# zhoujun-7/VPHO

Measured on AMD Instinct MI355X. Metric: eval images/sec (bs=64, sample_num=100, steps=50); MPJPE delta vs ref, higher is better.
Workload: dtype f32; 1 GPU; vpho_net.forward(mode=predict), README eval config (BASELINE.json configs[1]); per_gpu_batch=64, sample_num=100, sampling_steps=50, topk_hand=30, topk_obj=10, crop=256x256, pipeline_depth=3, parallelism=dp1, score_mfma=f32, conv_mfma=f32, winograd_3x3=True

## Files before the change

vpho_amd/csrc/common.h:

```cpp
#pragma once
#include <hip/hip_runtime.h>
#include <cstdio>
#include <cstdarg>

namespace vpho {
char* err_slot();
int fail(const char* fmt, ...);
inline int check_launch(const char* what) {
    hipError_t e = hipGetLastError();
    if (e != hipSuccess) return fail("%s: %s", what, hipGetErrorString(e));
    return 0;
}

enum ProfClass { PROF_CONV128 = 0, PROF_CONV64 = 1, PROF_SCORE_HEAD = 2, PROF_CONV128x64 = 3,
                 PROF_MANO_FK = 4, PROF_OBJ_PHYSICS = 5, PROF_HAND_FUSE = 6, PROF_ROI_ALIGN = 7, PROF_RESIZE = 8, PROF_WINOGRAD = 9,
                 PROF_WGRAD64 = 10, PROF_WGRAD128 = 11, PROF_FORCE_OPTIM = 12, PROF_POSE_ENC = 13, PROF_NCLASS = 14 };
bool prof_on(int cls);
void prof_record(int cls, hipEvent_t start, hipEvent_t stop, double flops, double bytes);
struct ProfScope {
    int cls; hipStream_t s; double flops, bytes; bool on; hipEvent_t e0, e1;
    ProfScope(int c, hipStream_t st, double f, double b = 0) : cls(c), s(st), flops(f), bytes(b), on(c >= 0 && prof_on(c)) {
        if (on) { (void)hipEventCreate(&e0); (void)hipEventCreate(&e1); (void)hipEventRecord(e0, s); }
    }
    ~ProfScope() { if (on) { (void)hipEventRecord(e1, s); prof_record(cls, e0, e1, flops, bytes); } }
};
int dynamic_lds(const void* kernel, int bytes);
}

#define VPHO_REQUIRE(cond, ...) do { if (!(cond)) return vpho::fail(__VA_ARGS__); } while (0)
#define VPHO_DYN_LDS(kernel, bytes) do { if (vpho::dynamic_lds(reinterpret_cast<const void*>(kernel), (int)(bytes))) return 1; } while (0)
#define VPHO_HIP(call) do { hipError_t e_ = (call); if (e_ != hipSuccess) return vpho::fail("%s: %s", #call, hipGetErrorString(e_)); } while (0)

#define VPHO_SYNC_LDS_DMA() do { asm volatile("s_waitcnt vmcnt(0)" ::: "memory"); __syncthreads(); } while (0)
#define VPHO_BARRIER_LDS_ONLY() asm volatile("s_waitcnt lgkmcnt(0)\n\ts_barrier" ::: "memory")

#ifndef VPHO_MAINLOOP_PRIO
#define VPHO_MAINLOOP_PRIO 0
#endif
#if VPHO_MAINLOOP_PRIO
#define VPHO_PRIO_MAIN() __builtin_amdgcn_s_setprio(VPHO_MAINLOOP_PRIO)
#define VPHO_PRIO_REST() __builtin_amdgcn_s_setprio(0)
#else
#define VPHO_PRIO_MAIN() ((void)0)
#define VPHO_PRIO_REST() ((void)0)
#endif

__device__ inline void lin_src(int dst, float scale, int in_size, int& i0, int& i1, float& l1) {
    float s = ((float)dst + 0.5f) * scale - 0.5f;
    s = s < 0.f ? 0.f : s;
    i0 = (int)s;
    i1 = i0 + (i0 < in_size - 1 ? 1 : 0);
    l1 = s - (float)i0;
}

#ifdef VPHO_CLOCK_STAMPS
#define VPHO_STAMP_SLOTS 65536
#define VPHO_STAMP_WORDS 10
#define VPHO_STAMP_DECL(name)                                                                                                      \
    __device__ unsigned long long name##_stamps[VPHO_STAMP_WORDS * VPHO_STAMP_SLOTS];                                              \
// ... 56 lines not shown
```

vpho_amd/csrc/mano.hip:

```cpp
#include "common.h"
#include "rot.h"
#include "../../include/vpho_hip.h"

namespace {

__constant__ int c_parent[16] = {-1, 0, 1, 2, 0, 4, 5, 0, 7, 8, 0, 10, 11, 0, 13, 14};
__constant__ int c_tips[5] = {745, 317, 444, 556, 673};
__constant__ int c_tips_ho3d[5] = {728, 353, 442, 576, 694};
__constant__ int c_order[21] = {0, 13, 14, 15, 16, 1, 2, 3, 17, 4, 5, 6, 18, 10, 11, 12, 19, 7, 8, 9, 20};
__constant__ int c_to_manolayer[21] = {0, 5, 6, 7, 9, 10, 11, 17, 18, 19, 13, 14, 15, 1, 2, 3, 4, 8, 12, 16, 20};

constexpr int NV = 778;

__global__ __launch_bounds__(256) void mano_shape_kernel(const vpho_mano_tables t, const float* __restrict__ betas, int n_img,
                                                         float* __restrict__ v_shaped, float* __restrict__ J) {
    __shared__ float vs[NV * 3];
    __shared__ float be[10];
    const int b = blockIdx.x;
    if (threadIdx.x < 10) be[threadIdx.x] = betas[b * 10 + threadIdx.x];
    __syncthreads();
    for (int i = threadIdx.x; i < NV * 3; i += blockDim.x) {
        float s = 0.f;
        for (int k = 0; k < 10; ++k) s += t.shapedirs[i * 10 + k] * be[k];
        s += t.v_template[i];
        vs[i] = s;
        v_shaped[(long long)b * NV * 3 + i] = s;
    }
    __syncthreads();
    const int wave = threadIdx.x >> 6, lane = threadIdx.x & 63;
    for (int o = wave; o < 48; o += 4) {
        const int j = o / 3, c = o % 3;
        float s = 0.f;
        for (int v = lane; v < NV; v += 64) s += t.J_regressor[j * NV + v] * vs[v * 3 + c];
        for (int off = 32; off > 0; off >>= 1) s += __shfl_xor(s, off);
        if (lane == 0) J[b * 48 + o] = s;
    }
}

struct FkArgs {
    vpho_mano_tables t;
    const float* pose; int ld_pose;
    const float* v_shaped; const float* J;
    long long n_hands; int hands_per_image;
    const unsigned char* ho3d;
    float* verts;
    float* joints;
};

template <int HB>
__global__ __launch_bounds__(256) void mano_fk_kernel(const FkArgs a) {
    __shared__ float R[HB][16][9];
    __shared__ float G[HB][16][12];
    __shared__ __attribute__((aligned(16))) float A[HB][16][12];
    __shared__ __attribute__((aligned(16))) float pmT[135][HB];
    __shared__ float jt[HB][21][3];
    __shared__ float tipv[HB][10][3];
    const int tid = threadIdx.x;
    const long long h0 = (long long)blockIdx.x * HB;
    auto hand_of = [&](int h) { const long long g = h0 + h; return g < a.n_hands ? g : a.n_hands - 1; };
    auto img_of = [&](int h) { return (int)(hand_of(h) / a.hands_per_image); };
    const int hj_h = tid >> 4, hj_j = tid & 15;
    const bool hj = tid < HB * 16;

    if (hj) {
        float r[9];
        vpho::mano_rodrigues(a.pose + hand_of(hj_h) * a.ld_pose + 3 * hj_j, r);
        for (int k = 0; k < 9; ++k) R[hj_h][hj_j][k] = r[k];
    }
    __syncthreads();
    for (int i = tid; i < HB * 135; i += 256) {
        const int h = i / 135, k = i - h * 135;
        const int e = k % 9;
        pmT[k][h] = R[h][k / 9 + 1][e] - ((e == 0 || e == 4 || e == 8) ? 1.f : 0.f);
    }
    for (int lvl = 0; lvl < 4; ++lvl) {
        if (hj && (hj_j == 0 ? 0 : (hj_j - 1) % 3 + 1) == lvl) {
            const float* Jr = a.J + img_of(hj_h) * 48;
            const int i = hj_j;
            float (*Gh)[12] = G[hj_h];
            const float* Ri = R[hj_h][i];
            if (i == 0) {
                for (int k = 0; k < 3; ++k) { for (int c = 0; c < 3; ++c) Gh[0][k * 4 + c] = Ri[k * 3 + c]; Gh[0][k * 4 + 3] = Jr[k]; }
            } else {
                const int p = c_parent[i];
                const float rel[3] = {Jr[i * 3 + 0] - Jr[p * 3 + 0], Jr[i * 3 + 1] - Jr[p * 3 + 1], Jr[i * 3 + 2] - Jr[p * 3 + 2]};
                for (int r = 0; r < 3; ++r) {
                    for (int c = 0; c < 3; ++c) {
                        float s = 0.f;
                        for (int k = 0; k < 3; ++k) s += Gh[p][r * 4 + k] * Ri[k * 3 + c];
                        Gh[i][r * 4 + c] = s;
                    }
                    float s = 0.f;
                    for (int k = 0; k < 3; ++k) s += Gh[p][r * 4 + k] * rel[k];
                    Gh[i][r * 4 + 3] = s + Gh[p][r * 4 + 3];
                }
            }
        }
        __syncthreads();
    }
    if (hj) {
        const float* Jr = a.J + img_of(hj_h) * 48;
        const int i = hj_j;
        for (int r = 0; r < 3; ++r) {
            float s = 0.f;
            for (int k = 0; k < 3; ++k) s += G[hj_h][i][r * 4 + k] * Jr[i * 3 + k];
            for (int c = 0; c < 3; ++c) A[hj_h][i][r * 4 + c] = G[hj_h][i][r * 4 + c];
            A[hj_h][i][r * 4 + 3] = G[hj_h][i][r * 4 + 3] - s;
            jt[hj_h][i][r] = G[hj_h][i][r * 4 + 3];
        }
    }
    __syncthreads();

    typedef float f32x2 __attribute__((ext_vector_type(2)));
    auto skin_tail = [&](int h, int v, const float* wv, const float* blend, float* out3) {
        const float* vsh = a.v_shaped + (long long)img_of(h) * NV * 3;
        float vp[3];
        for (int c = 0; c < 3; ++c) vp[c] = vsh[v * 3 + c] + blend[c];
        f32x2 T[6];
#pragma unroll
        for (int e = 0; e < 6; ++e) T[e] = f32x2{0.f, 0.f};
#pragma unroll
        for (int j = 0; j < 16; ++j) {
            const f32x2 w = {wv[j], wv[j]};
            const f32x2* Aj = reinterpret_cast<const f32x2*>(A[h][j]);
#pragma unroll
            for (int e = 0; e < 6; ++e) T[e] = __builtin_elementwise_fma(Aj[e], w, T[e]);
        }
        for (int r = 0; r < 3; ++r) out3[r] = fmaf(T[2 * r][0], vp[0], fmaf(T[2 * r][1], vp[1], fmaf(T[2 * r + 1][0], vp[2], T[2 * r + 1][1])));
    };
    auto fin = [](float v, float c) { return ((v - c) * 1000.f) / 1000.f; };

    if (blockIdx.y == 0) {
        for (int t = tid; t < HB * 10; t += 256) {
            const int h = t / 10, tip = t - h * 10;
            const int v = tip < 5 ? c_tips[tip] : c_tips_ho3d[tip - 5];
            float blend[3], wv[16], o[3];
            for (int c = 0; c < 3; ++c) {
                float s = 0.f;
                const float* pd = a.t.tip_posedirs_t ? a.t.tip_posedirs_t + tip * 3 + c : a.t.posedirs_t + v * 3 + c;
                const long long ld = a.t.tip_posedirs_t ? 30 : (long long)NV * 3;
                for (int k = 0; k < 135; ++k) s = fmaf(pd[k * ld], pmT[k][h], s);
                blend[c] = s;
            }
            for (int j = 0; j < 16; ++j) wv[j] = a.t.weights[v * 16 + j];
            skin_tail(h, v, wv, blend, o);
            for (int c = 0; c < 3; ++c) tipv[h][tip][c] = o[c];
            if (tip < 5) for (int c = 0; c < 3; ++c) jt[h][16 + tip][c] = o[c];
        }
        __syncthreads();
        for (int t = tid; t < HB * 21; t += 256) {
            const int h = t / 21, q = t - h * 21;
            if (h0 + h >= a.n_hands) continue;
            const bool ho = a.ho3d && a.ho3d[img_of(h)];
            const float cx = jt[h][0][0], cy = jt[h][0][1], cz = jt[h][0][2];
            const float* src;
            if (!ho) src = jt[h][c_order[q]];
            else if (q >= 16) src = tipv[h][5 + q - 16];
            else src = jt[h][c_order[c_to_manolayer[q]]];
            float* jo = a.joints + ((h0 + h) * 21 + q) * 3;
            jo[0] = fin(src[0], cx); jo[1] = fin(src[1], cy); jo[2] = fin(src[2], cz);
        }
    }
    if (a.verts) {
        const int v = (blockIdx.y * 4 + (tid >> 6)) * 64 + (tid & 63);
        if (v < NV) {
            float acc[HB][3];
            const float* pd = a.t.posedirs_t + v * 3;
            if constexpr (HB % 2 == 0) {
                f32x2 ap[HB / 2][3];
#pragma unroll
                for (int h = 0; h < HB / 2; ++h) ap[h][0] = ap[h][1] = ap[h][2] = f32x2{0.f, 0.f};
#pragma unroll 3
                for (int k = 0; k < 135; ++k) {
                    const float p0 = pd[(long long)k * NV * 3], p1 = pd[(long long)k * NV * 3 + 1], p2 = pd[(long long)k * NV * 3 + 2];
                    const f32x2 q0 = {p0, p0}, q1 = {p1, p1}, q2 = {p2, p2};
                    const f32x2* m2 = reinterpret_cast<const f32x2*>(pmT[k]);
#pragma unroll
// ... 241 lines not shown
                }
            __builtin_amdgcn_sched_barrier(0);
            if (v < NV) {
#pragma unroll
                for (int i = 0; i < 16; ++i) {
                    const int h = (i >> 2) * 8 + lh * 4 + (i & 3);
                    const float o = fmaf(T[0][i], acc[0][i], fmaf(T[1][i], acc[1][i], fmaf(T[2][i], acc[2][i], T[3][i])));
                    if ((FK_ABLATE & 1) && o != 1.2345e-30f) continue;
                    if (h0 + h < a.n_hands) a.verts[((h0 + h) * NV + v) * 3 + r] = fin(o, cen[i]);
                }
            }
            __builtin_amdgcn_sched_barrier(0);
        }
    }
}

}

extern "C" int vpho_mano_shape_f32(const vpho_mano_tables* t, const float* betas, int n_img, float* v_shaped, float* J, void* stream) {
    VPHO_REQUIRE(t && t->v_template && t->shapedirs && t->J_regressor && betas && v_shaped && J && n_img > 0, "vpho_mano_shape_f32: bad argument");
    hipLaunchKernelGGL(mano_shape_kernel, dim3(n_img), dim3(256), 0, (hipStream_t)stream, *t, betas, n_img, v_shaped, J);
    return vpho::check_launch("mano_shape_kernel");
}

extern "C" int vpho_mano_fk_f32(const vpho_mano_tables* t, const float* pose, int ld_pose, long long n_hands, int hands_per_image,
                                const float* v_shaped, const float* J, const unsigned char* ho3d_per_image,
                                float* verts, float* joints, void* stream) {
    VPHO_REQUIRE(t && t->posedirs_t && t->weights && pose && v_shaped && J && joints && n_hands > 0 && hands_per_image > 0 && ld_pose >= 48,
                 "vpho_mano_fk_f32: bad argument");
    VPHO_REQUIRE(n_hands < (1ll << 31), "vpho_mano_fk_f32: too many hands");
    FkArgs a;
    a.t = *t; a.pose = pose; a.ld_pose = ld_pose; a.v_shaped = v_shaped; a.J = J; a.n_hands = n_hands;
    a.hands_per_image = hands_per_image; a.ho3d = ho3d_per_image; a.verts = verts; a.joints = joints;
    const unsigned gy = verts ? 4 : 1;
    vpho::ProfScope prof(vpho::PROF_MANO_FK, (hipStream_t)stream, 0.0,
                         (double)n_hands * (48 * 4 + 21 * 12 + (verts ? 778 * 12 : 0)) + (double)((n_hands + hands_per_image - 1) / hands_per_image) * (778 + 16) * 12);
    static const bool no_mfma = getenv("VPHO_MANO_MFMA") && atoi(getenv("VPHO_MANO_MFMA")) == 0;
    if (verts && t->posedirs_mfma && n_hands >= 4096 && hands_per_image >= MH / 2 && !no_mfma) {
        VPHO_DYN_LDS(mano_fk_mfma_kernel, sizeof(FkMfmaLds));
        hipLaunchKernelGGL(mano_fk_mfma_kernel, dim3((unsigned)((n_hands + MH - 1) / MH)), dim3(512), sizeof(FkMfmaLds), (hipStream_t)stream, a);
        return vpho::check_launch("mano_fk_mfma_kernel");
    }
    if (n_hands >= 1024) hipLaunchKernelGGL(mano_fk_kernel<16>, dim3((unsigned)((n_hands + 15) / 16), gy), dim3(256), 0, (hipStream_t)stream, a);
    else if (n_hands >= 128) hipLaunchKernelGGL(mano_fk_kernel<4>, dim3((unsigned)((n_hands + 3) / 4), gy), dim3(256), 0, (hipStream_t)stream, a);
    else hipLaunchKernelGGL(mano_fk_kernel<1>, dim3((unsigned)n_hands, gy), dim3(256), 0, (hipStream_t)stream, a);
    return vpho::check_launch("mano_fk_kernel");
}
```

vpho_amd/csrc/misc.hip:

```cpp
#include "common.h"
#include <cstdint>
#include "rot.h"
#include "../../include/vpho_hip.h"

namespace {

inline int nblocks(long long n, int bs = 256) { return (int)((n + bs - 1) / bs); }

__global__ void nchw_to_nhwc_kernel(const float* __restrict__ x, int N, int C, int H, int W, float* __restrict__ y, int ldy) {
    const long long i = (long long)blockIdx.x * blockDim.x + threadIdx.x;
    const long long total = (long long)N * H * W * ldy;
    if (i >= total) return;
    const int c = (int)(i % ldy);
    const long long p = i / ldy;
    const long long hw = (long long)H * W;
    const long long n = p / hw, r = p - n * hw;
    y[i] = c < C ? x[(n * C + c) * hw + r] : 0.f;
}

__global__ void nhwc_to_nchw_kernel(const float* __restrict__ x, int N, int H, int W, int C, int ldx, float* __restrict__ y) {
    const long long i = (long long)blockIdx.x * blockDim.x + threadIdx.x;
    const long long hw = (long long)H * W, total = (long long)N * C * hw;
    if (i >= total) return;
    const long long r = i % hw;
    const long long nc = i / hw;
    const int c = (int)(nc % C);
    const long long n = nc / C;
    y[i] = x[(n * hw + r) * ldx + c];
}

__global__ void maxpool_nhwc_kernel(const float* __restrict__ x, int N, int H, int W, int C, int k, int stride, int pad,
                                    int OH, int OW, float* __restrict__ y) {
    const long long i = (long long)blockIdx.x * blockDim.x + threadIdx.x;
    const long long total = (long long)N * OH * OW * C;
    if (i >= total) return;
    const int c = (int)(i % C);
    long long p = i / C;
    const int ox = (int)(p % OW); p /= OW;
    const int oy = (int)(p % OH);
    const long long n = p / OH;
    float m = -INFINITY;
    for (int r = 0; r < k; ++r) {
        const int iy = oy * stride - pad + r;
        if (iy < 0 || iy >= H) continue;
        for (int s = 0; s < k; ++s) {
            const int ix = ox * stride - pad + s;
            if (ix < 0 || ix >= W) continue;
            m = fmaxf(m, x[((n * H + iy) * W + ix) * C + c]);
        }
    }
    y[i] = m;
}


template <int V>
__device__ inline void ldv(const float* __restrict__ p, float (&o)[V]) {
    if constexpr (V == 4) { const f32x4 t = *reinterpret_cast<const f32x4*>(p); o[0] = t[0]; o[1] = t[1]; o[2] = t[2]; o[3] = t[3]; }
    else o[0] = *p;
}
template <int V>
__device__ inline void stv(float* __restrict__ p, const float (&v)[V]) {
    if constexpr (V == 4) { f32x4 t; t[0] = v[0]; t[1] = v[1]; t[2] = v[2]; t[3] = v[3]; *reinterpret_cast<f32x4*>(p) = t; }
    else *p = v[0];
}

template <int V>
__global__ void resize_bilinear_nhwc_kernel(const float* __restrict__ x, int N, int H, int W, int C, int ldx, int OH, int OW,
                                            float* __restrict__ y, int ldy, int c_off, int accumulate,
                                            const int* __restrict__ row_map, const int* __restrict__ row_count) {
    const long long i = (long long)blockIdx.x * blockDim.x + threadIdx.x;
    const int CV = C / V;
    const long long total = (long long)N * OH * OW * CV;
    if (i >= total) return;
    const int c = (int)(i % CV) * V;
    long long p = i / CV;
    if (row_map) {
        if (p >= *row_count) return;
        p = row_map[p];
    }
    const int ox = (int)(p % OW); p /= OW;
    const int oy = (int)(p % OH);
    const long long n = p / OH;
    int y0, y1, x0, x1; float ly, lx;
    lin_src(oy, (float)H / (float)OH, H, y0, y1, ly);
// ... 407 lines not shown
    float* o = out + row * ldo + 3 * j;
    o[0] = aa[0]; o[1] = aa[1]; o[2] = aa[2];
}

__global__ void append_betas_kernel(const float* __restrict__ betas, long long rows, long long rows_per_image, float* __restrict__ out, int ldo) {
    const long long i = (long long)blockIdx.x * blockDim.x + threadIdx.x;
    if (i >= rows * 10) return;
    const long long row = i / 10;
    const int k = (int)(i - row * 10);
    out[row * ldo + 48 + k] = betas[(row / rows_per_image) * 10 + k];
}

}

#define LAUNCH1D(kernel, total, stream, ...) \
    hipLaunchKernelGGL(kernel, dim3(nblocks(total)), dim3(256), 0, (hipStream_t)(stream), __VA_ARGS__)

extern "C" int vpho_nchw_to_nhwc_f32(const float* x, int N, int C, int H, int W, float* y, int ldy, void* stream) {
    VPHO_REQUIRE(x && y && N > 0 && C > 0 && H > 0 && W > 0 && ldy >= C, "vpho_nchw_to_nhwc_f32: bad argument");
    LAUNCH1D(nchw_to_nhwc_kernel, (long long)N * H * W * ldy, stream, x, N, C, H, W, y, ldy);
    return vpho::check_launch("nchw_to_nhwc_kernel");
}

extern "C" int vpho_nhwc_to_nchw_f32(const float* x, int N, int H, int W, int C, int ldx, float* y, void* stream) {
    VPHO_REQUIRE(x && y && N > 0 && C > 0 && H > 0 && W > 0 && ldx >= C, "vpho_nhwc_to_nchw_f32: bad argument");
    LAUNCH1D(nhwc_to_nchw_kernel, (long long)N * H * W * C, stream, x, N, H, W, C, ldx, y);
    return vpho::check_launch("nhwc_to_nchw_kernel");
}

extern "C" int vpho_maxpool_nhwc_f32(const float* x, int N, int H, int W, int C, int k, int stride, int pad, float* y, void* stream) {
    VPHO_REQUIRE(x && y && N > 0 && C > 0 && k > 0 && stride > 0 && pad >= 0 && 2 * pad <= k, "vpho_maxpool_nhwc_f32: bad argument");
    const int OH = (H + 2 * pad - k) / stride + 1, OW = (W + 2 * pad - k) / stride + 1;
    VPHO_REQUIRE(OH > 0 && OW > 0, "vpho_maxpool_nhwc_f32: empty output");
    LAUNCH1D(maxpool_nhwc_kernel, (long long)N * OH * OW * C, stream, x, N, H, W, C, k, stride, pad, OH, OW, y);
    return vpho::check_launch("maxpool_nhwc_kernel");
}

extern "C" int vpho_resize_bilinear_nhwc_f32(const float* x, int N, int H, int W, int C, int ldx, int OH, int OW,
                                             float* y, int ldy, int c_off, int accumulate, void* stream) {
    VPHO_REQUIRE(x && y && N > 0 && C > 0 && H > 0 && W > 0 && OH > 0 && OW > 0 && ldx >= C && ldy >= c_off + C && c_off >= 0,
                 "vpho_resize_bilinear_nhwc_f32: bad argument");
    vpho::ProfScope prof(vpho::PROF_RESIZE, (hipStream_t)stream, 0.0, 4.0 * N * C * ((double)H * W + (double)OH * OW * (accumulate ? 2 : 1)));
    if (C % 4 == 0 && ldx % 4 == 0 && ldy % 4 == 0 && c_off % 4 == 0 && ((uintptr_t)x | (uintptr_t)y) % 16 == 0)
        LAUNCH1D(resize_bilinear_nhwc_kernel<4>, (long long)N * OH * OW * (C / 4), stream, x, N, H, W, C, ldx, OH, OW, y, ldy, c_off, accumulate, (const int*)nullptr, (const int*)nullptr);
    else
        LAUNCH1D(resize_bilinear_nhwc_kernel<1>, (long long)N * OH * OW * C, stream, x, N, H, W, C, ldx, OH, OW, y, ldy, c_off, accumulate, (const int*)nullptr, (const int*)nullptr);
    return vpho::check_launch("resize_bilinear_nhwc_kernel");
}

extern "C" int vpho_resize_bilinear_rows_nhwc_f32(const float* x, int N, int H, int W, int C, int ldx, int OH, int OW, float* y, int ldy, int c_off,
                                                  int accumulate, const int* row_map, const int* row_count, int rows_hint, void* stream) {
    VPHO_REQUIRE(x && y && row_map && row_count && N > 0 && H > 0 && W > 0 && C > 0 && OH > 0 && OW > 0 && ldx >= C && ldy >= c_off + C && c_off >= 0,
                 "vpho_resize_bilinear_rows_nhwc_f32: bad argument");
    const double px = rows_hint > 0 ? (double)rows_hint : (double)N * OH * OW;
    vpho::ProfScope prof(vpho::PROF_RESIZE, (hipStream_t)stream, 0.0, 4.0 * C * ((double)N * H * W + px * (accumulate ? 2 : 1)));
    if (C % 4 == 0 && ldx % 4 == 0 && ldy % 4 == 0 && c_off % 4 == 0 && ((uintptr_t)x | (uintptr_t)y) % 16 == 0)
        LAUNCH1D(resize_bilinear_nhwc_kernel<4>, (long long)N * OH * OW * (C / 4), stream, x, N, H, W, C, ldx, OH, OW, y, ldy, c_off, accumulate, row_map, row_count);
    else
        LAUNCH1D(resize_bilinear_nhwc_kernel<1>, (long long)N * OH * OW * C, stream, x, N, H, W, C, ldx, OH, OW, y, ldy, c_off, accumulate, row_map, row_count);
    return vpho::check_launch("resize_bilinear_nhwc_kernel(rows)");
}

extern "C" int vpho_roi_align_nhwc_f32(const float* feat, int N, int H, int W, int C, const float* boxes, float spatial_scale,
                                       int out_size, const unsigned char* flip_w, float* out, int ldo, int c_off, void* stream) {
    VPHO_REQUIRE(feat && boxes && out && N > 0 && C > 0 && out_size > 0 && ldo >= c_off + C && c_off >= 0, "vpho_roi_align_nhwc_f32: bad argument");
    vpho::ProfScope prof(vpho::PROF_ROI_ALIGN, (hipStream_t)stream, 0.0, 4.0 * N * C * ((double)H * W + (double)out_size * out_size));
// ... 85 lines not shown
    return vpho_mha_dropout_f32(qkv, S, B, E, nhead, nullptr, out, stream);
}

extern "C" int vpho_add_layernorm_f32(const float* x, const float* r, const float* gamma, const float* beta, long long rows, int E,
                                      float eps, float* out, void* stream) {
    VPHO_REQUIRE(x && r && gamma && beta && out && rows > 0 && E > 0, "vpho_add_layernorm_f32: bad argument");
    hipLaunchKernelGGL(add_layernorm_kernel, dim3((unsigned)((rows + 3) / 4)), dim3(256), 0, (hipStream_t)stream, x, r, gamma, beta, rows, E, eps, out);
    return vpho::check_launch("add_layernorm_kernel");
}

extern "C" int vpho_force_local_f32(const float* scale, int ld_scale, const float* logits, int ld_logits, const float* anchor,
                                    float friction, long long rows, int group, int group_stride, int off_scale, int off_logits,
                                    float* out, void* stream) {
    VPHO_REQUIRE(scale && logits && anchor && out && rows > 0 && ld_scale >= 1 && ld_logits >= 8 && group > 0 && group_stride >= group,
                 "vpho_force_local_f32: bad argument");
    LAUNCH1D(force_local_kernel, rows, stream, scale, ld_scale, logits, ld_logits, anchor, friction, rows, group, group_stride, off_scale, off_logits, out);
    return vpho::check_launch("force_local_kernel");
}

extern "C" int vpho_rot6d_to_axis_angle_f32(const float* x, long long rows, int rot_per_row, int ldx, float* out, int ldo, void* stream) {
    VPHO_REQUIRE(x && out && rows > 0 && rot_per_row > 0 && ldx >= 6 * rot_per_row && ldo >= 3 * rot_per_row, "vpho_rot6d_to_axis_angle_f32: bad argument");
    LAUNCH1D(rot6d_to_aa_kernel, rows * rot_per_row, stream, x, rows * rot_per_row, rot_per_row, ldx, out, ldo);
    return vpho::check_launch("rot6d_to_aa_kernel");
}

extern "C" int vpho_append_betas_f32(const float* betas, long long rows, long long rows_per_image, float* out, int ldo, void* stream) {
    VPHO_REQUIRE(betas && out && rows > 0 && rows_per_image > 0 && ldo >= 58, "vpho_append_betas_f32: bad argument");
    LAUNCH1D(append_betas_kernel, rows * 10, stream, betas, rows, rows_per_image, out, ldo);
    return vpho::check_launch("append_betas_kernel");
}


constexpr int LIN64_MAXK = 4096;
__global__ __launch_bounds__(256) void linear_acc64_kernel(const float* __restrict__ x, int rows, int K, int ld_x, const float* __restrict__ w,
                                                           const float* __restrict__ bias, int N, float slope, float* __restrict__ y, int ld_y) {
    const int n = blockIdx.x, lane = threadIdx.x & 63, wave = threadIdx.x >> 6;
    float wr[LIN64_MAXK / 64];
    const int nk = (K + 63) >> 6;
#pragma unroll
    for (int i = 0; i < LIN64_MAXK / 64; ++i) { const int k = i * 64 + lane; wr[i] = (i < nk && k < K) ? w[(long long)n * K + k] : 0.f; }
    const double b = bias ? (double)bias[n] : 0.0;
    for (int r = wave; r < rows; r += 4) {
        const float* xr = x + (long long)r * ld_x;
        double s = 0.0;
#pragma unroll
        for (int i = 0; i < LIN64_MAXK / 64; ++i) { const int k = i * 64 + lane; if (i < nk && k < K) s += (double)xr[k] * (double)wr[i]; }
        for (int off = 32; off > 0; off >>= 1) s += __shfl_xor(s, off);
        if (lane == 0) { const double v = s + b; y[(long long)r * ld_y + n] = (float)(v > 0.0 ? v : v * (double)slope); }
    }
}

extern "C" int vpho_linear_acc64_f32(const float* x, int rows, int cin, int ld_x, const float* w, const float* bias, int cout, float out_slope,
                                     float* y, int ld_y, void* stream) {
    VPHO_REQUIRE(x && w && y && rows > 0 && cin > 0 && cin <= LIN64_MAXK && cout > 0 && ld_x >= cin && ld_y >= cout, "vpho_linear_acc64_f32: bad argument (cin <= %d)", LIN64_MAXK);
    hipLaunchKernelGGL(linear_acc64_kernel, dim3(cout), dim3(256), 0, (hipStream_t)stream, x, rows, cin, ld_x, w, bias, cout, out_slope, y, ld_y);
    return vpho::check_launch("linear_acc64_kernel");
}
```

vpho_amd/csrc/score_ode.hip:

```cpp
#include "common.h"
#include <type_traits>
#include "../../include/vpho_hip.h"
#include <cmath>
#include <cstdlib>
#include <cstring>
#include <vector>
#include <mutex>
#include <unordered_map>
#include <algorithm>

VPHO_STAMP_DECL(head)

namespace {

#ifndef HEAD_ABLATE
#define HEAD_ABLATE 0
#endif
constexpr int HB_K = 16;
constexpr double SIGMA_MIN = 0.01, SIGMA_MAX = 50.0;

struct TimeList { float t[8]; };

struct RkCtl {
    double t, h_abs, h, t_new, err, dense_h;
    double T0, tf, rtol, atol, max_step, g_scale;
    double d[4];
    double *te, *dense_p, *log;
    int done, accepted, rejected, parity, kswap, status;
    int next_idx, num_steps, dense_first, dense_last, dense_parity, dense_kswap;
    int n_accepted, n_rejected, nfev, n_log, log_cap, n_attempts;
    float ts[8], inv_std[8], coef[8];
};
__device__ __host__ inline int kslot(int j, int kswap) { return (kswap && (j == 0 || j == 6)) ? 6 - j : j; }
__device__ inline bool ctl_skip(const RkCtl* ctl, int mode) {
    if (!ctl || mode == 0) return false;
    const int d = ctl->done;
    return mode == 1 ? d != 0 : d == 0;
}
__global__ __launch_bounds__(256) void time_embed_kernel(const vpho_score_weights w, TimeList tl, int NH, float* __restrict__ ct_all,
                                                         const RkCtl* __restrict__ ctl, int ctl_mode) {
    __shared__ float emb[128], tf[128];
    const int tid = threadIdx.x;
    if (ctl_skip(ctl, ctl_mode)) return;
    const float t = (ctl && ctl_mode == 1) ? ctl->ts[blockIdx.y] : tl.t[blockIdx.y];
    float* ct = ct_all + (long long)blockIdx.y * NH;
    if (tid < 64) {
        float a = t * w.t_W[tid];
        a = a * 2.0f;
        a = a * 3.14159265358979323846f;
        emb[tid] = sinf(a);
        emb[tid + 64] = cosf(a);
    }
    __syncthreads();
    if (tid < 128) {
        float s = 0.f;
        for (int i = 0; i < 128; ++i) s += w.t_w[tid * 128 + i] * emb[i];
        s += w.t_b[tid];
        tf[tid] = s > 0.f ? s : 0.f;
    }
    __syncthreads();
    const int o = blockIdx.x * 256 + tid;
    if (o < NH) {
        float s = 0.f;
        for (int k = 0; k < 128; ++k) s += tf[k] * w.w1_t[(long long)k * NH + o];
        ct[o] = s;
    }
}

struct LinComb { double c[7]; int n; double h; };
struct KSlots { const float* p[7]; };

struct PoseEncArgs {
    const float* X; int Dp;
    const double* y; KSlots ks; int D; LinComb lc; double* ynew; int use_lc;
    const float *w0, *b0, *w2, *b2;
    float* out; int R;
    const RkCtl* ctl; int ctl_mode, write_ynew; const float* kbase; long long n_el; double *ybuf0, *ybuf1;
};
constexpr int PE_ROWS = 32, PE_H_LD = 260, PE_NST = 3, PE_STAGE = 256 * 32;
__device__ __attribute__((aligned(256))) float g_pe_zero_page[64];

__global__ __launch_bounds__(512) void pose_encoder_kernel(const PoseEncArgs a) {
    extern __shared__ __attribute__((aligned(1024))) float smem[];
    const int K1 = (a.Dp + 31) / 32 * 32, X_LD = K1 + 4;
    float* Ws = smem;
    float* H1 = Ws + PE_NST * PE_STAGE;
    float* Bs = H1 + PE_ROWS * PE_H_LD;
    float* Xs = Bs + 512;
    const int tid = threadIdx.x, lane = tid & 63, wave = tid >> 6, li = lane & 31, lh = lane >> 5;
    const int r0 = blockIdx.x * PE_ROWS;
    const int n1 = K1 / 32, nch = n1 + 8;
    if (ctl_skip(a.ctl, a.ctl_mode)) return;
    KSlots ks = a.ks;
    const double* yv = a.y;
    double* ynew = a.ynew;
    double lch = a.lc.h;
    if (a.ctl && a.ctl_mode == 1 && a.use_lc) {
// ... 1233 lines not shown
    ws.bytes = off;
    return ws;
}

int check_weights(const vpho_score_weights* w) {
    VPHO_REQUIRE(w != nullptr, "score weights: null");
    VPHO_REQUIRE(w->nheads > 0 && w->D == w->nheads * 3 && w->Dp >= w->D && w->Dp % 4 == 0, "score weights: D=%d Dp=%d nheads=%d inconsistent", w->D, w->Dp, w->nheads);
    VPHO_REQUIRE(w->t_W && w->t_w && w->t_b && w->pe0_w && w->pe0_b && w->pe2_w && w->pe2_b && w->w1_t && w->w1_p && w->w1_f && w->b1 && w->w2 && w->b2, "score weights: null tensor");
    return 0;
}

int linear(const float* x, int rows, int cin, const float* wt, const float* bias, int cout, float slope, float* y, hipStream_t s) {
    vpho_conv_desc d;
    memset(&d, 0, sizeof(d));
    d.x = x; d.w = wt; d.bias = bias; d.y = y;
    d.N = rows; d.H = 1; d.W = 1; d.Cin = cin; d.x_ld = cin; d.Cout = cout; d.KH = 1; d.KW = 1; d.stride = 1;
    d.OH = 1; d.OW = 1; d.y_sx = cout; d.y_sy = cout; d.y_sn = cout; d.in_slope = 1.f; d.out_slope = slope;
    return vpho_conv2d_nhwc_f32(&d, s);
}

float sigma_f32(float t) { return (float)SIGMA_MIN * (float)std::pow(SIGMA_MAX / SIGMA_MIN, (double)t); }

struct Ctx {
    const vpho_score_weights* w; Workspace ws; int bs, S; long long R, n_el; int NH; hipStream_t s;
};

int prepare_cimg(Ctx& c, const float* feat_img) {
    return linear(feat_img, c.bs, 1024, c.w->w1_f, c.w->b1, c.NH, 1.f, c.ws.cimg, c.s);
}

int embed_times(Ctx& c, const float* ts, int n, int ctl_mode = 0) {
    TimeList tl;
    for (int i = 0; i < 8; ++i) tl.t[i] = (ts && i < n) ? ts[i] : 0.f;
    hipLaunchKernelGGL(time_embed_kernel, dim3((c.NH + 255) / 256, n), dim3(256), 0, c.s, *c.w, tl, c.NH, c.ws.ct,
                       ctl_mode ? c.ws.ctl : (const RkCtl*)nullptr, ctl_mode);
    return vpho::check_launch("time_embed_kernel");
}

struct CtlCall { int mode = 0, stage = 0, out_slot = 0, write_ynew = 0; };

int eval_net(Ctx& c, const float* X, float t, int rhs_mode, float coef, float* out, int ct_slot = -1,
             const LinComb* lc = nullptr, const double* y = nullptr, double* ynew = nullptr, const KSlots* ks = nullptr,
             CtlCall cc = CtlCall()) {
    if (ct_slot < 0) {
        if (int e = embed_times(c, &t, 1, cc.mode == 2 ? 2 : 0)) return e;
        ct_slot = 0;
    }
    {
        PoseEncArgs pa;
        memset(&pa, 0, sizeof(pa));
        pa.X = X; pa.Dp = c.w->Dp; pa.w0 = c.w->pe0_w; pa.b0 = c.w->pe0_b; pa.w2 = c.w->pe2_w; pa.b2 = c.w->pe2_b;
        pa.out = c.ws.P2; pa.R = (int)c.R;
        if (lc) { pa.use_lc = 1; pa.lc = *lc; pa.y = y; if (ks) pa.ks = *ks; pa.D = c.w->D; pa.ynew = ynew; }
        pa.ctl = cc.mode ? c.ws.ctl : nullptr; pa.ctl_mode = cc.mode; pa.write_ynew = cc.write_ynew; pa.kbase = c.ws.K; pa.n_el = c.n_el;
        pa.ybuf0 = c.ws.y; pa.ybuf1 = c.ws.ynew;
        const int K1 = (pa.Dp + 31) / 32 * 32;
        const char* pe_env = getenv("VPHO_PE_RING");
        const bool pe_ring = pe_env && atoi(pe_env);
        const dim3 pe_grid((unsigned)((c.R + PE_ROWS - 1) / PE_ROWS));
        vpho::ProfScope pe_prof(vpho::PROF_POSE_ENC, c.s, 2.0 * (double)c.R * 256.0 * (K1 + 256.0), 0.0);
        if (pe_ring) {
            const size_t pe_lds = (size_t)(PE_NST * PE_STAGE + PE_ROWS * PE_H_LD + 512 + PE_ROWS * (K1 + 4)) * sizeof(float);
            VPHO_DYN_LDS(pose_encoder_kernel, 150 * 1024);
            VPHO_REQUIRE(pe_lds <= 150 * 1024, "pose encoder: input dimension %d too large for the LDS tile", pa.Dp);
            hipLaunchKernelGGL(pose_encoder_kernel, pe_grid, dim3(512), pe_lds, c.s, pa);
        } else {
// ... 486 lines not shown
```

Measured before the change: 2234 images/s.

## Optimize leaf kernels: vectorized maxpool, tiled fp64 linear, staged time-embed and FK tips

Adds faster versions of several small leaf kernels, with an env var (VPHO_LEAF_REF) that selects the old reference kernels. Maxpool gains a float4-vectorized path. The fp64-accumulating linear now computes a 4x4 row/column tile per wave instead of one output column per block. Time embedding stages its weights through LDS with vector loads and preloads the w1 column into registers. MANO FK stages the tip posedirs into a shared union buffer, and the FKJ_ABLATE ablation macros default to off. These mostly cut redundant global loads and improve coalescing in small kernels, at the cost of more registers and LDS.

```diff
diff --git a/vpho_amd/csrc/common.h b/vpho_amd/csrc/common.h
--- a/vpho_amd/csrc/common.h
+++ b/vpho_amd/csrc/common.h
@@ -2,6 +2,7 @@
 #include <hip/hip_runtime.h>
 #include <cstdio>
 #include <cstdarg>
+#include <cstdlib>
 
 namespace vpho {
 char* err_slot();
@@ -25,6 +26,7 @@
     ~ProfScope() { if (on) { (void)hipEventRecord(e1, s); prof_record(cls, e0, e1, flops, bytes); } }
 };
 int dynamic_lds(const void* kernel, int bytes);
+inline bool leaf_ref() { const char* e = getenv("VPHO_LEAF_REF"); return e && e[0] == '1'; }
 }
 
 #define VPHO_REQUIRE(cond, ...) do { if (!(cond)) return vpho::fail(__VA_ARGS__); } while (0)
diff --git a/vpho_amd/csrc/mano.hip b/vpho_amd/csrc/mano.hip
--- a/vpho_amd/csrc/mano.hip
+++ b/vpho_amd/csrc/mano.hip
@@ -45,12 +45,17 @@
     const unsigned char* ho3d;
     float* verts;
     float* joints;
+    int tips_direct;
 };
 
+#ifndef FKJ_ABLATE
+#define FKJ_ABLATE 0
+#endif
 template <int HB>
 __global__ __launch_bounds__(256) void mano_fk_kernel(const FkArgs a) {
-    __shared__ float R[HB][16][9];
-    __shared__ float G[HB][16][12];
+    __shared__ union { struct { float R[HB][16][9]; float G[HB][16][12]; } kin; float tippd[135][30]; } u;
+    float (&R)[HB][16][9] = u.kin.R;
+    float (&G)[HB][16][12] = u.kin.G;
     __shared__ __attribute__((aligned(16))) float A[HB][16][12];
     __shared__ __attribute__((aligned(16))) float pmT[135][HB];
     __shared__ float jt[HB][21][3];
@@ -62,9 +67,22 @@
     const int hj_h = tid >> 4, hj_j = tid & 15;
     const bool hj = tid < HB * 16;
 
+    constexpr int TIP_W = (135 * 30 + 255) / 256;
+    const bool stage_tips = blockIdx.y == 0 && !a.tips_direct;
+    float tipw[TIP_W];
+    if (stage_tips) {
+#pragma unroll
+        for (int q = 0; q < TIP_W; ++q) {
+            const int i = min(q * 256 + tid, 135 * 30 - 1), k = i / 30, col = i - k * 30, tip = col / 3;
+            tipw[q] = a.t.tip_posedirs_t ? a.t.tip_posedirs_t[i]
+                                         : a.t.posedirs_t[(long long)k * NV * 3 + (tip < 5 ? c_tips[tip] : c_tips_ho3d[tip - 5]) * 3 + (col - tip * 3)];
+        }
+    }
+
     if (hj) {
         float r[9];
-        vpho::mano_rodrigues(a.pose + hand_of(hj_h) * a.ld_pose + 3 * hj_j, r);
+        if (FKJ_ABLATE & 8) { for (int k = 0; k < 9; ++k) r[k] = 0.1f * (float)(k + hj_j); }
+        else vpho::mano_rodrigues(a.pose + hand_of(hj_h) * a.ld_pose + 3 * hj_j, r);
         for (int k = 0; k < 9; ++k) R[hj_h][hj_j][k] = r[k];
     }
     __syncthreads();
@@ -73,7 +91,7 @@
         const int e = k % 9;
         pmT[k][h] = R[h][k / 9 + 1][e] - ((e == 0 || e == 4 || e == 8) ? 1.f : 0.f);
     }
-    for (int lvl = 0; lvl < 4; ++lvl) {
+    for (int lvl = 0; lvl < ((FKJ_ABLATE & 1) ? 0 : 4); ++lvl) {
         if (hj && (hj_j == 0 ? 0 : (hj_j - 1) % 3 + 1) == lvl) {
             const float* Jr = a.J + img_of(hj_h) * 48;
             const int i = hj_j;
@@ -131,18 +149,31 @@
     auto fin = [](float v, float c) { return ((v - c) * 1000.f) / 1000.f; };
 
     if (blockIdx.y == 0) {
-        for (int t = tid; t < HB * 10; t += 256) {
+        if (stage_tips) {
+#pragma unroll
+            for (int q = 0; q < TIP_W; ++q)
+                if (q * 256 + tid < 135 * 30) (&u.tippd[0][0])[q * 256 + tid] = tipw[q];
+            __syncthreads();
+        }
+        for (int t = tid; t < ((FKJ_ABLATE & 2) ? 0 : HB * 10); t += 256) {
             const int h = t / 10, tip = t - h * 10;
             const int v = tip < 5 ? c_tips[tip] : c_tips_ho3d[tip - 5];
             float blend[3], wv[16], o[3];
-            for (int c = 0; c < 3; ++c) {
+            if (stage_tips) {
+                blend[0] = blend[1] = blend[2] = 0.f;
+                for (int k = 0; k < 135; ++k) {
+                    const float m = pmT[k][h];
+#pragma unroll
+                    for (int c = 0; c < 3; ++c) blend[c] = fmaf((FKJ_ABLATE & 4) ? 0.25f : u.tippd[k][tip * 3 + c], m, blend[c]);
+                }
+            } else for (int c = 0; c < 3; ++c) {
                 float s = 0.f;
                 const float* pd = a.t.tip_posedirs_t ? a.t.tip_posedirs_t + tip * 3 + c : a.t.posedirs_t + v * 3 + c;
                 const long long ld = a.t.tip_posedirs_t ? 30 : (long long)NV * 3;
-                for (int k = 0; k < 135; ++k) s = fmaf(pd[k * ld], pmT[k][h], s);
+                for (int k = 0; k < 135; ++k) s = fmaf((FKJ_ABLATE & 4) ? 0.25f : pd[k * ld], pmT[k][h], s);
                 blend[c] = s;
             }
-            for (int j = 0; j < 16; ++j) wv[j] = a.t.weights[v * 16 + j];
+            for (int j = 0; j < 16; ++j) wv[j] = (FKJ_ABLATE & 4) ? 0.0625f : a.t.weights[v * 16 + j];
             skin_tail(h, v, wv, blend, o);
             for (int c = 0; c < 3; ++c) tipv[h][tip][c] = o[c];
             if (tip < 5) for (int c = 0; c < 3; ++c) jt[h][16 + tip][c] = o[c];
@@ -450,6 +481,7 @@
     FkArgs a;
     a.t = *t; a.pose = pose; a.ld_pose = ld_pose; a.v_shaped = v_shaped; a.J = J; a.n_hands = n_hands;
     a.hands_per_image = hands_per_image; a.ho3d = ho3d_per_image; a.verts = verts; a.joints = joints;
+    a.tips_direct = vpho::leaf_ref();
     const unsigned gy = verts ? 4 : 1;
     vpho::ProfScope prof(vpho::PROF_MANO_FK, (hipStream_t)stream, 0.0,
                          (double)n_hands * (48 * 4 + 21 * 12 + (verts ? 778 * 12 : 0)) + (double)((n_hands + hands_per_image - 1) / hands_per_image) * (778 + 16) * 12);
diff --git a/vpho_amd/csrc/misc.hip b/vpho_amd/csrc/misc.hip
--- a/vpho_amd/csrc/misc.hip
+++ b/vpho_amd/csrc/misc.hip
@@ -50,6 +50,31 @@
         }
     }
     y[i] = m;
+}
+
+__global__ __launch_bounds__(256) void maxpool_nhwc_kernel_v4(const float* __restrict__ x, int H, int W, int C4, int k, int stride, int pad,
+                                                              int OH, int OW, unsigned total, float* __restrict__ y) {
+    const unsigned i = blockIdx.x * 256u + threadIdx.x;
+    if (i >= total) return;
+    const unsigned c4 = i % (unsigned)C4;
+    unsigned p = i / (unsigned)C4;
+    const int ox = (int)(p % (unsigned)OW); p /= (unsigned)OW;
+    const int oy = (int)(p % (unsigned)OH);
+    const unsigned n = p / (unsigned)OH;
+    const f32x4* __restrict__ x4 = reinterpret_cast<const f32x4*>(x);
+    f32x4 m = {-INFINITY, -INFINITY, -INFINITY, -INFINITY};
+    for (int r = 0; r < k; ++r) {
+        const int iy = oy * stride - pad + r;
+        if (iy < 0 || iy >= H) continue;
+        const unsigned row = (n * (unsigned)H + (unsigned)iy) * (unsigned)W;
+        for (int s = 0; s < k; ++s) {
+            const int ix = ox * stride - pad + s;
+            if (ix < 0 || ix >= W) continue;
+            const f32x4 v = x4[(row + (unsigned)ix) * (unsigned)C4 + c4];
+            m[0] = fmaxf(m[0], v[0]); m[1] = fmaxf(m[1], v[1]); m[2] = fmaxf(m[2], v[2]); m[3] = fmaxf(m[3], v[3]);
+        }
+    }
+    reinterpret_cast<f32x4*>(y)[i] = m;
 }
 
 
@@ -523,6 +548,12 @@
     VPHO_REQUIRE(x && y && N > 0 && C > 0 && k > 0 && stride > 0 && pad >= 0 && 2 * pad <= k, "vpho_maxpool_nhwc_f32: bad argument");
     const int OH = (H + 2 * pad - k) / stride + 1, OW = (W + 2 * pad - k) / stride + 1;
     VPHO_REQUIRE(OH > 0 && OW > 0, "vpho_maxpool_nhwc_f32: empty output");
+    const long long n_in = (long long)N * H * W * C, n_out = (long long)N * OH * OW * C;
+    if (C % 4 == 0 && (((uintptr_t)x | (uintptr_t)y) & 15) == 0 && n_in < (1LL << 31) && n_out < (1LL << 31) && !vpho::leaf_ref()) {
+        hipLaunchKernelGGL(maxpool_nhwc_kernel_v4, dim3(nblocks(n_out / 4)), dim3(256), 0, (hipStream_t)stream, x, H, W, C / 4, k, stride, pad,
+                           OH, OW, (unsigned)(n_out / 4), y);
+        return vpho::check_launch("maxpool_nhwc_kernel_v4");
+    }
     LAUNCH1D(maxpool_nhwc_kernel, (long long)N * OH * OW * C, stream, x, N, H, W, C, k, stride, pad, OH, OW, y);
     return vpho::check_launch("maxpool_nhwc_kernel");
 }
@@ -674,7 +705,7 @@
 
 
 constexpr int LIN64_MAXK = 4096;
-__global__ __launch_bounds__(256) void linear_acc64_kernel(const float* __restrict__ x, int rows, int K, int ld_x, const float* __restrict__ w,
+__global__ __launch_bounds__(256) void linear_acc64_ref_kernel(const float* __restrict__ x, int rows, int K, int ld_x, const float* __restrict__ w,
                                                            const float* __restrict__ bias, int N, float slope, float* __restrict__ y, int ld_y) {
     const int n = blockIdx.x, lane = threadIdx.x & 63, wave = threadIdx.x >> 6;
     float wr[LIN64_MAXK / 64];
@@ -692,9 +723,68 @@
     }
 }
 
+constexpr int LIN64_RB = 4, LIN64_CB = 4;
+__global__ __launch_bounds__(256) void linear_acc64_kernel(const float* __restrict__ x, int rows, int K, int ld_x, const float* __restrict__ w,
+                                                           const float* __restrict__ bias, int N, float slope, float* __restrict__ y, int ld_y) {
+    const int lane = threadIdx.x & 63, wave = threadIdx.x >> 6;
+    const int n0 = blockIdx.x * LIN64_CB, r0 = (blockIdx.y * 4 + wave) * LIN64_RB;
+    if (r0 >= rows) return;
+    const float* xp[LIN64_RB];
+    const float* wp[LIN64_CB];
+#pragma unroll
+    for (int r = 0; r < LIN64_RB; ++r) xp[r] = x + (long long)min(r0 + r, rows - 1) * ld_x + lane;
+#pragma unroll
+    for (int c = 0; c < LIN64_CB; ++c) wp[c] = w + (long long)min(n0 + c, N - 1) * K + lane;
+    double acc[LIN64_RB][LIN64_CB];
+#pragma unroll
+    for (int r = 0; r < LIN64_RB; ++r)
+#pragma unroll
+        for (int c = 0; c < LIN64_CB; ++c) acc[r][c] = 0.0;
+    const int nfull = K >> 6;
+#pragma unroll 2
+    for (int i = 0; i < nfull; ++i) {
+        double xv[LIN64_RB], wv[LIN64_CB];
+#pragma unroll
+        for (int r = 0; r < LIN64_RB; ++r) xv[r] = (double)xp[r][i * 64];
+#pragma unroll
+        for (int c = 0; c < LIN64_CB; ++c) wv[c] = (double)wp[c][i * 64];
+#pragma unroll
+        for (int r = 0; r < LIN64_RB; ++r)
+#pragma unroll
+            for (int c = 0; c < LIN64_CB; ++c) acc[r][c] += xv[r] * wv[c];
+    }
+    if (nfull * 64 + lane < K) {
+#pragma unroll
+        for (int r = 0; r < LIN64_RB; ++r)
+#pragma unroll
+            for (int c = 0; c < LIN64_CB; ++c) acc[r][c] += (double)xp[r][nfull * 64] * (double)wp[c][nfull * 64];
+    }
+    for (int off = 32; off > 0; off >>= 1) {
+#pragma unroll
+        for (int r = 0; r < LIN64_RB; ++r)
+#pragma unroll
+            for (int c = 0; c < LIN64_CB; ++c) acc[r][c] += __shfl_xor(acc[r][c], off);
+    }
+    double s = 0.0;
+#pragma unroll
+    for (int r = 0; r < LIN64_RB; ++r)
+#pragma unroll
+        for (int c = 0; c < LIN64_CB; ++c) s = lane == r * LIN64_CB + c ? acc[r][c] : s;
+    const int r = r0 + lane / LIN64_CB, n = n0 + lane % LIN64_CB;
+    if (lane < LIN64_RB * LIN64_CB && r < rows && n < N) {
+        const double v = s + (bias ? (double)bias[n] : 0.0);
+        y[(long long)r * ld_y + n] = (float)(v > 0.0 ? v : v * (double)slope);
+    }
+}
+
 extern "C" int vpho_linear_acc64_f32(const float* x, int rows, int cin, int ld_x, const float* w, const float* bias, int cout, float out_slope,
                                      float* y, int ld_y, void* stream) {
     VPHO_REQUIRE(x && w && y && rows > 0 && cin > 0 && cin <= LIN64_MAXK && cout > 0 && ld_x >= cin && ld_y >= cout, "vpho_linear_acc64_f32: bad argument (cin <= %d)", LIN64_MAXK);
-    hipLaunchKernelGGL(linear_acc64_kernel, dim3(cout), dim3(256), 0, (hipStream_t)stream, x, rows, cin, ld_x, w, bias, cout, out_slope, y, ld_y);
+    if (vpho::leaf_ref()) {
+        hipLaunchKernelGGL(linear_acc64_ref_kernel, dim3(cout), dim3(256), 0, (hipStream_t)stream, x, rows, cin, ld_x, w, bias, cout, out_slope, y, ld_y);
+        return vpho::check_launch("linear_acc64_ref_kernel");
+    }
+    hipLaunchKernelGGL(linear_acc64_kernel, dim3((cout + LIN64_CB - 1) / LIN64_CB, (rows + 4 * LIN64_RB - 1) / (4 * LIN64_RB)), dim3(256), 0,
+                       (hipStream_t)stream, x, rows, cin, ld_x, w, bias, cout, out_slope, y, ld_y);
     return vpho::check_launch("linear_acc64_kernel");
 }
diff --git a/vpho_amd/csrc/score_ode.hip b/vpho_amd/csrc/score_ode.hip
--- a/vpho_amd/csrc/score_ode.hip
+++ b/vpho_amd/csrc/score_ode.hip
@@ -3,6 +3,7 @@
 #include "../../include/vpho_hip.h"
 #include <cmath>
 #include <cstdlib>
+#include <cstdint>
 #include <cstring>
 #include <vector>
 #include <mutex>
@@ -37,8 +38,8 @@
     const int d = ctl->done;
     return mode == 1 ? d != 0 : d == 0;
 }
-__global__ __launch_bounds__(256) void time_embed_kernel(const vpho_score_weights w, TimeList tl, int NH, float* __restrict__ ct_all,
-                                                         const RkCtl* __restrict__ ctl, int ctl_mode) {
+__global__ __launch_bounds__(256) void time_embed_ref_kernel(const vpho_score_weights w, TimeList tl, int NH, float* __restrict__ ct_all,
+                                                             const RkCtl* __restrict__ ctl, int ctl_mode) {
     __shared__ float emb[128], tf[128];
     const int tid = threadIdx.x;
     if (ctl_skip(ctl, ctl_mode)) return;
@@ -63,6 +64,59 @@
     if (o < NH) {
         float s = 0.f;
         for (int k = 0; k < 128; ++k) s += tf[k] * w.w1_t[(long long)k * NH + o];
+        ct[o] = s;
+    }
+}
+
+constexpr int TE_LD = 132;
+__global__ __launch_bounds__(256) void time_embed_kernel(const vpho_score_weights w, TimeList tl, int NH, float* __restrict__ ct_all,
+                                                         const RkCtl* __restrict__ ctl, int ctl_mode) {
+    __shared__ __attribute__((aligned(16))) float tw[128 * TE_LD];
+    __shared__ __attribute__((aligned(16))) float emb[128];
+    __shared__ float tf[128];
+    const int tid = threadIdx.x;
+    if (ctl_skip(ctl, ctl_mode)) return;
+    const float t = (ctl && ctl_mode == 1) ? ctl->ts[blockIdx.y] : tl.t[blockIdx.y];
+    float* ct = ct_all + (long long)blockIdx.y * NH;
+    f32x4 stage[16];
+    const f32x4* __restrict__ tw4 = reinterpret_cast<const f32x4*>(w.t_w);
+#pragma unroll
+    for (int q = 0; q < 16; ++q) stage[q] = tw4[q * 256 + tid];
+    const int o = blockIdx.x * 256 + tid;
+    const float* __restrict__ w1c = w.w1_t + (o < NH ? o : NH - 1);
+    float w1v[128];
+#pragma unroll
+    for (int k = 0; k < 128; ++k) w1v[k] = w1c[(long long)k * NH];
+    if (tid < 64) {
+        float a = t * w.t_W[tid];
+        a = a * 2.0f;
+        a = a * 3.14159265358979323846f;
+        emb[tid] = sinf(a);
+        emb[tid + 64] = cosf(a);
+    }
+#pragma unroll
+    for (int q = 0; q < 16; ++q) {
+        const int f = q * 256 + tid;
+        *reinterpret_cast<f32x4*>(tw + (f >> 5) * TE_LD + (f & 31) * 4) = stage[q];
+    }
+    __syncthreads();
+    if (tid < 128) {
+        const f32x4* __restrict__ row = reinterpret_cast<const f32x4*>(tw + tid * TE_LD);
+        const f32x4* __restrict__ e4 = reinterpret_cast<const f32x4*>(emb);
+        float s = 0.f;
+#pragma unroll 8
+        for (int j = 0; j < 32; ++j) {
+            const f32x4 a = row[j], e = e4[j];
+            s += a[0] * e[0]; s += a[1] * e[1]; s += a[2] * e[2]; s += a[3] * e[3];
+        }
+        s += w.t_b[tid];
+        tf[tid] = s > 0.f ? s : 0.f;
+    }
+    __syncthreads();
+    if (o < NH) {
+        float s = 0.f;
+#pragma unroll
+        for (int k = 0; k < 128; ++k) s += tf[k] * w1v[k];
         ct[o] = s;
     }
 }
@@ -1362,6 +1416,11 @@
 int embed_times(Ctx& c, const float* ts, int n, int ctl_mode = 0) {
     TimeList tl;
     for (int i = 0; i < 8; ++i) tl.t[i] = (ts && i < n) ? ts[i] : 0.f;
+    if (vpho::leaf_ref() || ((uintptr_t)c.w->t_w & 15)) {
+        hipLaunchKernelGGL(time_embed_ref_kernel, dim3((c.NH + 255) / 256, n), dim3(256), 0, c.s, *c.w, tl, c.NH, c.ws.ct,
+                           ctl_mode ? c.ws.ctl : (const RkCtl*)nullptr, ctl_mode);
+        return vpho::check_launch("time_embed_ref_kernel");
+    }
     hipLaunchKernelGGL(time_embed_kernel, dim3((c.NH + 255) / 256, n), dim3(256), 0, c.s, *c.w, tl, c.NH, c.ws.ct,
                        ctl_mode ? c.ws.ctl : (const RkCtl*)nullptr, ctl_mode);
     return vpho::check_launch("time_embed_kernel");
```

After: 2095 images/s. -6.2%, worse.
